# zhengfei0908/SBA-GAN

Hardware: AMD Instinct MI355X
Metric: images/sec (G+D step) at 256px (higher is better)
Workload: dtype bf16; 1 GPU; bird_style.yml 3-stage G+D step (64..256px), B=20 per GPU, G_NET variant=model, image_encoder=inception, text_encoder=RNN_ENCODER in the step; global_batch=20, parallelism=dp1, launch=replayer, losses_finite=True

## Files before the change

### include/sbagan_hip.h

```cpp
#ifndef SBAGAN_HIP_H
#define SBAGAN_HIP_H

#include <stdint.h>

#ifdef __cplusplus
extern "C" {
#endif

#define SBA_F32 0
#define SBA_BF16 1
#define SBA_BF16_YH 2

#define SBA_OK 0
#define SBA_E_ARG (-1)
#define SBA_E_LAUNCH (-2)
#define SBA_E_UNSUPPORTED (-3)

#define SBA_ACT_NONE 0
#define SBA_ACT_GLU 1
#define SBA_ACT_LRELU 2
#define SBA_ACT_RELU 3

#define SBA_MAX_TAPS 32

typedef struct sba_conv_geom {
    int32_t N, IH, IW, Cin;
    int32_t OH, OW, Cout;
    int32_t OHs, OWs;
    int32_t sy, sx;
    int32_t osy, osx, ooy, oox;
    int32_t ups;
    int32_t ntaps;
    int8_t ty[SBA_MAX_TAPS];
    int8_t tx[SBA_MAX_TAPS];
    int32_t x_cstride, x_coff, y_cstride, y_coff;
    int32_t relu;
    int32_t tile, ksplit;
    int32_t first_write;
    int32_t w_layout;
} sba_conv_geom;
#define SBA_IGEMM_TILES 18

const char* sba_version(void);

int sba_set_deterministic(int on, void* scratch, int64_t scratch_bytes);
int sba_get_deterministic(void);
int sba_det_reset(void);
int64_t sba_det_high_water(void);
int sba_set_reduce_scratch(void* scratch, int64_t scratch_bytes);
int sba_bn_stat_slots(void);

int sba_conv_igemm(int dtype, const void* x, const void* w, void* y, const void* addend,
                   float* stats, const sba_conv_geom* g, void* workspace, int64_t workspace_bytes,
                   void* stream);
int sba_conv_igemm_bias(int dtype, const void* x, const void* w, void* y, const void* addend,
                        float* stats, const float* bias, const void* relu_mask, const sba_conv_geom* g,
                        void* workspace, int64_t workspace_bytes, void* stream);
int sba_conv_igemm_plan(int dtype, const sba_conv_geom* g, int64_t workspace_bytes, int* plan);
int sba_conv_igemm_tile_shape(int tile, int* bm, int* bn);

int sba_fold_bn_pack(int dtype, const float* w, const float* gamma, const float* beta, const float* running_mean,
                     const float* running_var, float eps, void* out, float* bias, int O, int taps, int Cin, int glu,
                     void* stream);
int sba_conv_igemm_glu(int dtype, const void* x, const void* w, const float* bias, void* y, int C,
                       const sba_conv_geom* g, void* stream);
int sba_conv_igemm_glu_plan(int dtype, const sba_conv_geom* g, int C, int* plan);
#define SBA_GROUP_MAX 8
typedef struct sba_conv_group_item {
    const void* x; const void* w; void* y; const void* addend; const float* bias; const void* relu_mask;
    const sba_conv_geom* g;
} sba_conv_group_item;
int sba_conv_igemm_group(int dtype, int n, const sba_conv_group_item* items, int tile, void* stream);
int sba_conv_igemm_group_splitk(int dtype, int n, const sba_conv_group_item* items, int tile, int ksplit,
                                void* workspace, int64_t workspace_bytes, void* stream);
int sba_conv_wgrad(int dtype, const void* x, const void* dy, float* dw, const sba_conv_geom* g,
                   int ksplit, void* stream);
#define SBA_WGRAD_PLAN_INTS 14
int sba_conv_wgrad_plan(int dtype, const sba_conv_geom* g, int ksplit, int det, int* plan);
int sba_pack_weight(int dtype, const float* w, void* out, int Cout, int KH, int KW, int Cin,
                    int mode, void* stream);
typedef struct sba_pack_desc {
    const float* w;
    void* fwd;
    void* tr;
    int32_t Cout, KH, KW, Cin;
    int32_t mode;
    int32_t tile_begin;
    int32_t co_tiles, ci_tiles;
} sba_pack_desc;
int sba_pack_weights_multi(int dtype, const sba_pack_desc* descs, int ndesc, int total_tiles, void* stream);
typedef struct sba_frag_desc {
    const void* src;
    void* dst;
    int32_t R, taps, K, unit_begin;
} sba_frag_desc;
int sba_pack_frag_multi(const sba_frag_desc* descs, int ndesc, int total_units, void* stream);
int sba_pool2x2_sum(int dtype, const void* dup, void* dx, int N, int H, int W, int C, void* stream);

#ifndef SBA_BN_STAT_SLOTS
#define SBA_BN_STAT_SLOTS 8
#endif
int sba_bn_stats(int dtype, const void* y, float* stats, int64_t rows, int groups, int C, void* stream);
int sba_bn_act_fwd(int dtype, const void* y, const float* stats, const float* gamma, const float* beta,
                   float* running_mean, float* running_var, int64_t* num_batches_tracked, float* aux,
                   const void* residual, void* out, int64_t rows, int groups, int C, int act,
                   int out_cstride, int out_coff, float eps, float momentum, int training, void* stream);
int sba_bn_act_bwd_reduce(int dtype, const void* y, const void* dout, const float* aux, float* red,
                          int64_t rows, int groups, int C, int act, int dout_cstride, int dout_coff,
                          void* stream);
int sba_bn_act_bwd_apply(int dtype, const void* y, const void* dout, const float* aux, const float* red,
                         void* dy, float* dgamma, float* dbeta, int64_t rows, int groups, int C, int act,
                         int dout_cstride, int dout_coff, void* stream);
int sba_bn_act_fwd_fused(int dtype, const void* y, const float* gamma, const float* beta, float* running_mean,
                         float* running_var, int64_t* num_batches_tracked, float* aux, void* out, int64_t rows,
                         int groups, int C, int act, int out_cstride, int out_coff, float eps, float momentum,
                         void* stream);
int sba_bn_act_bwd_fused(int dtype, const void* y, const void* dout, const float* aux, void* dy,
                         float* dgamma, float* dbeta, int64_t rows, int groups, int C, int act,
                         int dout_cstride, int dout_coff, void* stream);
int sba_bn1d_glu_fwd(int dtype, const float* y, const float* gamma, const float* beta,
                     float* running_mean, float* running_var, int64_t* nbt, float* mean,
                     float* rstd, void* out, int B, int F, float eps, float momentum, void* stream);
int sba_bn1d_glu_bwd(int dtype, const float* y, const void* dout, const float* gamma,
                     const float* beta, const float* mean, const float* rstd, float* dy,
                     float* dgamma, float* dbeta, int B, int F, void* stream);

int sba_linear_fwd(const float* x, const float* w, const float* bias, float* y, int B, int K, int N,
                   void* stream);
int sba_linear_glu_fwd(int dtype, const float* x, const float* wp, const float* bias, void* out, int B, int K,
                       int F2, void* stream);
int sba_linear_bwd(const float* x, const float* w, const float* dy, float* dx, float* dw,
                   float* dbias, int B, int K, int N, void* stream);
int sba_ca_fwd(const float* h, const float* eps, float* c, float* mu, float* logvar, int B, int C,
               void* stream);
int sba_ca_bwd(const float* h, const float* eps, const float* dc, const float* dmu,
               const float* dlogvar, float* dh, int B, int C, void* stream);

int sba_ctx_proj_fwd(const float* words, const float* W, float* src, int B, int idf, int cdf, int L,
                     void* stream);
int sba_ctx_proj_fwd_fp8(const float* words, const float* W, float* src, int B, int idf, int cdf, int L,
                         void* stream);
int sba_ctx_proj_bwd(const float* words, const float* W, const float* dsrc, float* dW, float* dwords,
                     int B, int idf, int cdf, int L, void* stream);

int sba_instnorm_stats(int dtype, const void* h, float* mean, float* rstd, int N, int HW, int C,
                       float eps, void* stream);
int sba_adain_fwd(int dtype, const void* h, const float* mean, const float* rstd, const float* style,
                  void* out, int N, int HW, int C, int out_cstride, int out_coff, void* stream);
int sba_adain_bwd_reduce(int dtype, const void* h, const void* dout, const float* mean,
                         const float* rstd, float* red, int N, int HW, int C, int dout_cstride,
                         int dout_coff, void* stream);
int sba_adain_bwd_apply(int dtype, const void* h, const void* dout, const float* mean,
                        const float* rstd, const float* style, const float* red, void* dh,
                        float* dstyle, int N, int HW, int C, int dout_cstride, int dout_coff,
                        int accumulate, void* stream);

int sba_word_attn_fwd(int dtype, const void* h, const float* src, const uint8_t* mask, void* ctx,
                      float* att, int B, int Q, int idf, int L, int mask_mode, int out_cstride,
                      int out_coff, void* stream);
int sba_word_attn_fwd_fp8(const void* h, const float* src, const uint8_t* mask, void* ctx, float* att, int B, int Q,
                          int idf, int L, int mask_mode, int out_cstride, int out_coff, void* stream);
int sba_word_attn_bwd(int dtype, const void* h, const float* src, const uint8_t* mask,
                      const void* dctx, void* dh, float* dsrc, int B, int Q, int idf, int L,
                      int mask_mode, int dctx_cstride, int dctx_coff, int accumulate, void* stream);

int sba_img_head_fwd(int dtype, const void* h, const float* w, float* img, int N, int H, int W,
                     int C, void* stream);
int sba_img_head_bwd(int dtype, const void* h, const float* w, const float* img, const float* dimg,
                     void* dh, float* dw, int N, int H, int W, int C, int accumulate, void* stream);

int sba_d_stem_fwd(int dtype, const float* img, const float* w, void* out, int N, int S, int C,
                   void* stream);
int sba_d_stem_bwd(int dtype, const float* img, const float* w, const void* out, const void* dout,
                   float* dimg, float* dw, int N, int S, int C, void* stream);

int sba_logits_fwd(int dtype, const void* h, const float* w, const float* bias, float* prob, int B,
                   int K, void* stream);
int sba_logits_bwd(int dtype, const void* h, const float* w, const float* prob, const float* dprob,
                   void* dh, float* dw, float* dbias, int B, int K, int accumulate, void* stream);
int sba_cond_cat_fwd(int dtype, const void* h, const float* sent, void* out, int B, int C, int E,
                     void* stream);
int sba_cond_cat_bwd(int dtype, const void* dout, void* dh, float* dsent, int B, int C, int E,
                     int accumulate, void* stream);

int sba_resize_bilinear(const float* in, float* out, int NC, int S, int D, int backward, void* stream);
int sba_enc_stem_fwd(int dtype, const float* img, const float* w, const float* bias, void* out, int N, int S, int C,
                     void* stream);
int sba_enc_stem_bwd(int dtype, const float* w, const void* out, const void* dout, float* dimg, int N, int S, int C,
                     void* stream);
int sba_enc_stem_resize_fwd(int dtype, const float* img, const float* w, const float* bias, void* out, int N, int S, int D,
                            int C, void* stream);
int sba_maxpool3x3s2_fwd(int dtype, const void* x, void* y, int N, int H, int W, int C, int xcs, int xco, int ycs,
                         int yco, void* stream);
int sba_maxpool3x3s2_bwd(int dtype, const void* x, const void* dy, void* dx, int N, int H, int W, int C, int xcs,
                         int xco, int dycs, int dyco, int dxcs, int dxco, int accumulate, void* stream);
int sba_maxpool3x3s2_fwd_arg(int dtype, const void* x, void* y, uint8_t* argmax, int N, int H, int W, int C, int xcs,
                             int xco, int ycs, int yco, void* stream);
int sba_maxpool3x3s2_bwd_arg(int dtype, const uint8_t* argmax, const void* dy, void* dx, int N, int H, int W, int C,
                             int dycs, int dyco, int dxcs, int dxco, int accumulate, const void* relu_mask, void* stream);
int sba_avgpool3x3(int dtype, const void* x, void* y, int N, int H, int W, int C, int xcs, int xco, int ycs, int yco,
                   int accumulate, void* stream);
int sba_relu_bwd(int dtype, const void* out, const void* dout, void* dpre, int64_t rows, int C, int ocs, int oco,
                 int dcs, int dco, void* stream);
int sba_global_avgpool(int dtype, void* x, float* y, int N, int HW, int C, int backward, void* stream);
int sba_layout_nhwc_nchw(int dtype, void* nhwc, float* nchw, int N, int HW, int C, int to_nhwc, void* stream);

int sba_bce_multi(const float* prob, const int32_t* offsets, const float* target, const float* weight,
                  int nseg, float* loss, float* dprob, void* stream);
int sba_kl_loss(const float* mu, const float* logvar, float* loss, float* dmu, float* dlogvar,
                int n, void* stream);
int sba_damsm_words_fwd(const float* feat, const float* words, const int64_t* cap_lens, float* sim,
                        float* attn, float* attn1, float* wctx, int B, int nef, int R, int L,
                        float gamma1, float gamma2, void* stream);
int sba_damsm_words_bwd(const float* feat, const float* words, const int64_t* cap_lens,
                        const float* sim, const float* attn, const float* attn1, const float* wctx,
                        const float* dsim, float* dfeat, float* dwords, int B, int nef, int R, int L,
                        float gamma1, float gamma2, void* stream);
int64_t sba_damsm_prep_bytes(int B, int nef, int R, int L);
int64_t sba_damsm_bwd_bytes(int B, int nef, int R, int L);
int sba_damsm_prep(const float* feat, const float* words, const int64_t* cap_lens, void* prep, int64_t prep_bytes,
                   int B, int nef, int R, int L, void* stream);
int sba_damsm_words_fwd_mfma(const void* prep, const float* words, const int64_t* cap_lens, float* sim, float* attn,
                             float* attn1, float* wctx, int B, int nef, int R, int L, float gamma1, float gamma2,
                             void* stream);
int sba_damsm_words_bwd_mfma(const void* prep, const float* words, const int64_t* cap_lens, const float* sim,
                             const float* attn, const float* attn1, const float* wctx, const float* dsim,
                             void* scratch, int64_t scratch_bytes, float* dfeat, int accumulate, float* dwords,
                             int B, int nef, int R, int L, float gamma1, float gamma2, void* stream);
int sba_ce_pair_direct(const float* score, const uint8_t* mask, float scale, float lam, float* loss_out,
                       float* dscore, int B, void* stream);
int sba_damsm_sent_direct(const float* cnn, const float* rnn, const uint8_t* mask, float gamma3, float eps, float lam,
// ... 73 lines not shown
```

### sba-gan_amd/csrc/wgrad.hip

```cpp
#include "common.h"
#include "conv_common.h"

namespace {

struct FastDiv {
    uint64_t magic;
    uint32_t d;
};
static inline FastDiv make_fastdiv(uint32_t d, int64_t max_n) {
    FastDiv f;
    f.d = d;
    f.magic = (max_n < (1 << 21) && d > 0) ? (((uint64_t)1 << 42) + d - 1) / d : 0;
    return f;
}
__device__ __forceinline__ uint32_t fdiv(uint32_t n, const FastDiv& f) {
    return f.magic ? (uint32_t)(((uint64_t)n * f.magic) >> 42) : n / f.d;
}

__device__ __forceinline__ void zero_acc(f32x16_t (&acc)[2][2]) {
#pragma unroll
    for (int i = 0; i < 2; ++i)
#pragma unroll
        for (int j = 0; j < 2; ++j)
#pragma unroll
// ... 698 lines not shown
    for (int kw = 0; kw < 3; ++kw)
        store_tile<false>(acc[kw], dw + (int64_t)blockIdx.z * zstride, g, co0, ci0, kh * 3 + kw, mode, lane);
}

enum WgradFamily { WG_ROW_DMA = 0, WG_SMALL_DMA = 1, WG_SMALL = 2, WG_ROWS = 3, WG_GENERIC = 4 };

struct WgradPlan {
    int family;
    int v[4];
    dim3 grid;
    int block, lds;
    int per_split;
    int mode;
    int npart;
    int wclog;
};

static int pixel_splits(int target_wgs, int wgs, int chunks, int min_chunks, int* per_split) {
    int sp = cdiv(target_wgs, wgs);
    if (sp > chunks / min_chunks) sp = chunks / min_chunks > 0 ? chunks / min_chunks : 1;
    *per_split = cdiv(chunks, sp);
    return cdiv(chunks, *per_split);
}

static bool wgrad_plan(int dtype, const sba_conv_geom* g, int ksplit, bool det_on, WgradPlan* p) {
    if (!geom_ok(g, dtype)) return false;
    if (g->Cin % 8 != 0 || g->Cout % 8 != 0) return false;
    if (g->x_cstride || g->x_coff || g->y_cstride || g->y_coff || g->ntaps > 16) return false;
    const int M = g->N * g->OHs * g->OWs;
    if (ksplit < 1) ksplit = 1;
    const int fw = g->first_write ? 2 : 0;
    const int co_tiles = cdiv(g->Cout, 64), items = cdiv(g->Cin, 64) * g->ntaps;
    const bool dma_ok = dtype == SBA_BF16 && (int64_t)g->N * g->OH * g->OW * g->Cout * 2 < (1ll << 32);
    auto fill = [&](int family, int v0, int v1, int v2, int v3, dim3 grid, int block, int lds, int per_split, int unsplit_mode) {
        *p = WgradPlan{family, {v0, v1, v2, v3}, grid, block, lds, per_split, 0, 0, 0};
        const int nz = (int)grid.z;
        p->npart = det_on && (nz > 1 || family == WG_ROWS) ? nz : 0;
        p->mode = p->npart ? 2 : (nz > 1 ? 1 : unsplit_mode);
        return grid.y <= 65535 && grid.z <= 65535;
    };
    {
        const int kwn = g->ntaps == 16 ? 4 : (g->ntaps == 9 ? 3 : 0), sxy = g->sx;
        bool ok = dma_ok && kwn && g->sy == sxy && (!g->ups || kwn == 3) && g->osy == 1 && g->osx == 1 && g->ooy == 0 &&
                  g->oox == 0 && g->OHs == g->OH && g->OWs == g->OW && g->Cin % 64 == 0 && g->Cout % 64 == 0 &&
                  g->OW >= 4 && (g->OW & (g->OW - 1)) == 0 && !(g->OW == 4 && (g->ups || g->OH != 4)) && M % 32 == 0 &&
                  ((g->OH * g->OW) % 32 == 0 || g->OW == 4);
        ok = ok && ((kwn == 4 && sxy == 2) || (kwn == 3 && sxy == 1));
        for (int t = 0; t < g->ntaps && ok; ++t)
            ok = g->ty[t] == g->ty[(t / kwn) * kwn] && g->tx[t] == g->tx[(t / kwn) * kwn] + (t % kwn);
        if (ok) {
            const int wc = g->OW < 32 ? g->OW : 32;
            int wclog = 0;
            while ((1 << wclog) < wc) ++wclog;
            const int wgs = co_tiles * kwn * (g->Cin / 64);
            constexpr int ROW_WGS = 512;
            int cps32;
            const int sp = pixel_splits(wgs <= 8 ? (ROW_WGS * 3) / 4 : ROW_WGS, wgs, M / 32, 12, &cps32);
            const int xb = kwn == 4 ? 10 : (g->OW == 4 ? 6 : 5);
            const int stage = kwn == 4 ? WgRowCfg<4, 10>::STAGE : (g->OW == 4 ? WgRowCfg<3, 6>::STAGE : WgRowCfg<3, 5>::STAGE);
            if (fill(WG_ROW_DMA, kwn, sxy, xb, 4, dim3(co_tiles, kwn * (g->Cin / 64), sp), 64 * kwn, 4 * stage, cps32, fw)) {
                p->wclog = wclog;
                return true;
            }
        }
    }
    constexpr int SMALL_M = 12000;
    if (M <= SMALL_M && co_tiles * items >= 256) {
        const int wgs = co_tiles * cdiv(items, 4);
        constexpr int SMALL_WGS = 768, SMALL_MINC = 24;
        const int target = wgs >= SMALL_WGS / 2 ? wgs : SMALL_WGS;
        int cps;
        const int split = pixel_splits(target, wgs, cdiv(M, 16), SMALL_MINC, &cps);
        const dim3 grid(co_tiles, cdiv(items, 4), split);
        if (grid.y > 65535 || grid.z > 65535) return false;
        constexpr int DMA_WGS = 512;
        if (fw == 2 && wgs > DMA_WGS && g->Cout % 128 == 0 && dma_ok) {
            fill(WG_SMALL_DMA, 2, 3, 0, 0, dim3(co_tiles / 2, cdiv(items, 4), 1), 256, 3 * 6 * 32 * 128, cdiv(M, 32), fw);
            return true;
        }
        if (wgs <= DMA_WGS && dma_ok) {
            int cps32;
            const int sp = pixel_splits(target, wgs, cdiv(M, 32), SMALL_MINC / 2, &cps32);
            return fill(WG_SMALL_DMA, 1, 4, 0, 0, dim3(co_tiles, cdiv(items, 4), sp), 256, 4 * 5 * 32 * 128, cps32, fw);
        }
        return fill(WG_SMALL, dtype, 0, 0, 0, grid, 256, 0, cps, fw);
    }
    constexpr int ROWS_M = 131072;
    bool rows_ok = g->ntaps == 9 && g->sy == 1 && g->sx == 1 && g->osy == 1 && g->osx == 1 && g->ooy == 0 &&
                   g->oox == 0 && g->OHs == g->OH && g->OWs == g->OW && g->OW % 64 == 0 && M >= ROWS_M;
    for (int t = 0; t < 9 && rows_ok; ++t) rows_ok = g->ty[t] == t / 3 - 1 && g->tx[t] == t % 3 - 1;
    if (rows_ok) {
        const int ci_t = cdiv(g->Cin, 64);
        int spw;
        const int nz = pixel_splits(256, co_tiles * ci_t, g->N * g->OH * (g->OW / 64), 16, &spw);
        return fill(WG_ROWS, dtype, 0, 0, 0, dim3(co_tiles, ci_t, nz), 192, 0, spw, 1);
    }
    if (dma_ok) {
        constexpr int GEN_WGS = 512;
        int cps32;
        const int sp = pixel_splits(GEN_WGS, co_tiles * cdiv(items, 4), cdiv(M, 32), 12, &cps32);
        if (fill(WG_SMALL_DMA, 1, 4, 0, 0, dim3(co_tiles, cdiv(items, 4), sp), 256, 4 * 5 * 32 * 128, cps32, fw)) return true;
    }
    const int total_chunks = cdiv(M, 64);
    if (ksplit > total_chunks) ksplit = total_chunks;
    const int cps = cdiv(total_chunks, ksplit);
    return fill(WG_GENERIC, dtype, 0, 0, 0, dim3(co_tiles, items, cdiv(total_chunks, cps)), 256, 0, cps, 0);
}

template <auto Kernel, typename... Args>
static void launch_dyn_lds(const WgradPlan& p, hipStream_t st, Args... args) {
    static bool once = false;
    if (!once) { (void)hipFuncSetAttribute((const void*)Kernel, hipFuncAttributeMaxDynamicSharedMemorySize, p.lds); once = true; }
    SBA_LAUNCH(Kernel, p.grid, dim3(p.block), p.lds, st, args...);
}

static int wgrad_launch(const WgradPlan& p, int dtype, const void* x, const void* dy, float* dw, const sba_conv_geom* g,
                        hipStream_t st) {
    const int M = g->N * g->OHs * g->OWs;
    const FastDiv dsub = make_fastdiv((uint32_t)(g->OHs * g->OWs), (int64_t)M + 64);
    const FastDiv dow = make_fastdiv((uint32_t)g->OWs, (int64_t)M + 64);
    const int64_t dwn = (int64_t)g->Cout * g->ntaps * g->Cin;
    float* part = nullptr;
    if (p.npart) { part = sba_det_alloc((int64_t)p.npart * dwn); if (!part) return SBA_E_ARG; }
    float* dwa = part ? part : dw;
    const int64_t zs = part ? dwn : 0;
    const bf16_t* xh = (const bf16_t*)x;
    const bf16_t* dyh = (const bf16_t*)dy;
    switch (p.family) {
    case WG_ROW_DMA:
        if (p.v[0] == 4) launch_dyn_lds<wgrad_row_dma_kernel<4, 2, 10, 4>>(p, st, xh, dyh, dwa, *g, M, p.per_split, p.mode, dsub, dow, zs, p.wclog);
        else if (p.v[2] == 6) launch_dyn_lds<wgrad_row_dma_kernel<3, 1, 6, 4>>(p, st, xh, dyh, dwa, *g, M, p.per_split, p.mode, dsub, dow, zs, p.wclog);
        else launch_dyn_lds<wgrad_row_dma_kernel<3, 1, 5, 4>>(p, st, xh, dyh, dwa, *g, M, p.per_split, p.mode, dsub, dow, zs, p.wclog);
        break;
    case WG_SMALL_DMA:
        if (p.v[0] == 2) launch_dyn_lds<wgrad_small_dma_kernel<2, 3>>(p, st, xh, dyh, dwa, *g, M, p.per_split, p.mode, dsub, dow, zs);
        else launch_dyn_lds<wgrad_small_dma_kernel<1, 4>>(p, st, xh, dyh, dwa, *g, M, p.per_split, p.mode, dsub, dow, zs);
        break;
    case WG_SMALL:
        SBA_DISPATCH(dtype, SBA_LAUNCH((wgrad_small_kernel<T>), p.grid, dim3(p.block), 0, st, (const T*)x, (const T*)dy, dwa, *g, M,
                                       p.per_split, p.mode, dsub, dow, zs));
        break;
    case WG_ROWS:
        SBA_DISPATCH(dtype, SBA_LAUNCH((wgrad_rows_kernel<T>), p.grid, dim3(p.block), 0, st, (const T*)x, (const T*)dy, dwa, *g,
                                       g->N * g->OH * (g->OW / 64), p.per_split, p.mode, zs));
        break;
    default:
        SBA_DISPATCH(dtype, SBA_LAUNCH((wgrad_kernel<T>), p.grid, dim3(p.block), 0, st, (const T*)x, (const T*)dy, dwa, *g, M,
                                       p.per_split, p.mode, dsub, dow, zs));
    }
    if (part) sba_det_fold(part, 1, p.npart, dwn, dw, 0, g->first_write ? 1 : 0, st);
    return SBA_CHECK_LAUNCH();
}

}

extern "C" int sba_conv_wgrad_plan(int dtype, const sba_conv_geom* g, int ksplit, int det, int* plan) {
    WgradPlan p;
    if (!plan || !wgrad_plan(dtype, g, ksplit, det != 0, &p)) return SBA_E_ARG;
    const int out[SBA_WGRAD_PLAN_INTS] = {p.family, p.v[0], p.v[1], p.v[2], p.v[3], (int)p.grid.x, (int)p.grid.y, (int)p.grid.z,
                                          p.block, p.lds, p.per_split, p.mode, p.npart, p.wclog};
    for (int i = 0; i < SBA_WGRAD_PLAN_INTS; ++i) plan[i] = out[i];
    return SBA_OK;
}

extern "C" int sba_conv_wgrad(int dtype, const void* x, const void* dy, float* dw, const sba_conv_geom* g,
                              int ksplit, void* stream) {
    WgradPlan p;
    if (!x || !dy || !dw || !wgrad_plan(dtype, g, ksplit, sba_det_on(), &p)) return SBA_E_ARG;
    return wgrad_launch(p, dtype, x, dy, dw, g, (hipStream_t)stream);
}
```

### sba-gan_amd/sbagan/_lib.py

```python
import ctypes
import os

import torch
from ctypes import (POINTER, Structure, byref, c_char_p, c_float, c_int, c_int8, c_int32, c_int64,
                    c_uint64, c_void_p)

_HERE = os.path.dirname(os.path.abspath(__file__))
LIB_PATH = os.environ.get('SBA_LIB_PATH') or os.path.join(os.path.dirname(_HERE), 'csrc', 'libsbagan_hip.so')

SBA_F32, SBA_BF16, SBA_BF16_YH = 0, 1, 2
IGEMM_TILES = 18
WGRAD_PLAN_INTS = 14
WGRAD_FAMILIES = ('row_dma', 'small_dma', 'small', 'rows', 'generic')
ACT_NONE, ACT_GLU, ACT_LRELU, ACT_RELU = 0, 1, 2, 3
MAX_TAPS = 32


class ConvGeom(Structure):
    _fields_ = [('N', c_int32), ('IH', c_int32), ('IW', c_int32), ('Cin', c_int32),
                ('OH', c_int32), ('OW', c_int32), ('Cout', c_int32),
                ('OHs', c_int32), ('OWs', c_int32),
                ('sy', c_int32), ('sx', c_int32),
                ('osy', c_int32), ('osx', c_int32), ('ooy', c_int32), ('oox', c_int32),
                ('ups', c_int32), ('ntaps', c_int32),
                ('ty', c_int8 * MAX_TAPS), ('tx', c_int8 * MAX_TAPS),
                ('x_cstride', c_int32), ('x_coff', c_int32), ('y_cstride', c_int32), ('y_coff', c_int32),
                ('relu', c_int32), ('tile', c_int32), ('ksplit', c_int32), ('first_write', c_int32),
                ('w_layout', c_int32)]


class ConvGroupItem(Structure):
    _fields_ = [('x', c_void_p), ('w', c_void_p), ('y', c_void_p), ('addend', c_void_p), ('bias', c_void_p),
                ('relu_mask', c_void_p), ('g', POINTER(ConvGeom))]


GROUP_MAX = 8

if not os.path.exists(LIB_PATH):
    raise ImportError('libsbagan_hip.so not built: run `python __graft_entry__.py` or '
                      '`make -C sba-gan_amd/csrc` (expected %s)' % LIB_PATH)
lib = ctypes.CDLL(LIB_PATH)

P, I, F, L, U = c_void_p, c_int, c_float, c_int64, c_uint64
G = POINTER(ConvGeom)

SIGNATURES = {
    'sba_conv_igemm': [I, P, P, P, P, P, G, P, L, P],
    'sba_conv_igemm_bias': [I, P, P, P, P, P, P, P, G, P, L, P],
    'sba_conv_igemm_plan': [I, G, L, POINTER(c_int)],
    'sba_conv_igemm_tile_shape': [I, POINTER(c_int), POINTER(c_int)],
    'sba_fold_bn_pack': [I, P, P, P, P, P, F, P, P, I, I, I, I, P],
    'sba_conv_igemm_glu': [I, P, P, P, P, I, G, P],
    'sba_conv_igemm_glu_plan': [I, G, I, POINTER(c_int)],
    'sba_conv_igemm_group': [I, I, POINTER(ConvGroupItem), I, P],
    'sba_conv_igemm_group_splitk': [I, I, POINTER(ConvGroupItem), I, I, P, L, P],
    'sba_conv_wgrad': [I, P, P, P, G, I, P],
    'sba_conv_wgrad_plan': [I, G, I, I, POINTER(c_int)],
    'sba_pack_weight': [I, P, P, I, I, I, I, I, P],
    'sba_pack_frag_multi': [P, I, I, P],
    'sba_pack_weights_multi': [I, P, I, I, P],
    'sba_pool2x2_sum': [I, P, P, I, I, I, I, P],
    'sba_bn_stats': [I, P, P, L, I, I, P],
    'sba_bn_act_fwd': [I, P, P, P, P, P, P, P, P, P, P, L, I, I, I, I, I, F, F, I, P],
    'sba_bn_act_bwd_reduce': [I, P, P, P, P, L, I, I, I, I, I, P],
    'sba_bn_act_fwd_fused': [I, P, P, P, P, P, P, P, P, L, I, I, I, I, I, F, F, P],
    'sba_bn_act_bwd_fused': [I, P, P, P, P, P, P, L, I, I, I, I, I, P],
    'sba_bn_act_bwd_apply': [I, P, P, P, P, P, P, P, L, I, I, I, I, I, P],
    'sba_bn1d_glu_fwd': [I, P, P, P, P, P, P, P, P, P, I, I, F, F, P],
    'sba_bn1d_glu_bwd': [I, P, P, P, P, P, P, P, P, P, I, I, P],
    'sba_linear_fwd': [P, P, P, P, I, I, I, P],
    'sba_linear_glu_fwd': [I, P, P, P, P, I, I, I, P],
    'sba_linear_bwd': [P, P, P, P, P, P, I, I, I, P],
    'sba_ca_fwd': [P, P, P, P, P, I, I, P],
    'sba_ca_bwd': [P, P, P, P, P, P, I, I, P],
    'sba_ctx_proj_fwd': [P, P, P, I, I, I, I, P],
    'sba_ctx_proj_bwd': [P, P, P, P, P, I, I, I, I, P],
    'sba_ctx_proj_fwd_fp8': [P, P, P, I, I, I, I, P],
    'sba_instnorm_stats': [I, P, P, P, I, I, I, F, P],
    'sba_adain_fwd': [I, P, P, P, P, P, I, I, I, I, I, P],
    'sba_adain_bwd_reduce': [I, P, P, P, P, P, I, I, I, I, I, P],
    'sba_adain_bwd_apply': [I, P, P, P, P, P, P, P, P, I, I, I, I, I, I, P],
    'sba_word_attn_fwd': [I, P, P, P, P, P, I, I, I, I, I, I, I, P],
    'sba_word_attn_fwd_fp8': [P, P, P, P, P, I, I, I, I, I, I, I, P],
    'sba_word_attn_bwd': [I, P, P, P, P, P, P, I, I, I, I, I, I, I, I, P],
    'sba_img_head_fwd': [I, P, P, P, I, I, I, I, P],
    'sba_img_head_bwd': [I, P, P, P, P, P, P, I, I, I, I, I, P],
    'sba_d_stem_fwd': [I, P, P, P, I, I, I, P],
    'sba_d_stem_bwd': [I, P, P, P, P, P, P, I, I, I, P],
    'sba_logits_fwd': [I, P, P, P, P, I, I, P],
    'sba_logits_bwd': [I, P, P, P, P, P, P, P, I, I, I, P],
    'sba_cond_cat_fwd': [I, P, P, P, I, I, I, P],
    'sba_cond_cat_bwd': [I, P, P, P, I, I, I, I, P],
    'sba_resize_bilinear': [P, P, I, I, I, I, P],
    'sba_enc_stem_fwd': [I, P, P, P, P, I, I, I, P],
    'sba_enc_stem_resize_fwd': [I, P, P, P, P, I, I, I, I, P],
    'sba_enc_stem_bwd': [I, P, P, P, P, I, I, I, P],
    'sba_maxpool3x3s2_fwd': [I, P, P, I, I, I, I, I, I, I, I, P],
    'sba_maxpool3x3s2_bwd': [I, P, P, P, I, I, I, I, I, I, I, I, I, I, I, P],
    'sba_maxpool3x3s2_fwd_arg': [I, P, P, P, I, I, I, I, I, I, I, I, P],
    'sba_maxpool3x3s2_bwd_arg': [I, P, P, P, I, I, I, I, I, I, I, I, I, P, P],
    'sba_avgpool3x3': [I, P, P, I, I, I, I, I, I, I, I, I, P],
    'sba_relu_bwd': [I, P, P, P, L, I, I, I, I, I, P],
    'sba_global_avgpool': [I, P, P, I, I, I, I, P],
    'sba_layout_nhwc_nchw': [I, P, P, I, I, I, I, P],
    'sba_bce_multi': [P, P, P, P, I, P, P, P],
    'sba_kl_loss': [P, P, P, P, P, I, P],
    'sba_damsm_words_fwd': [P, P, P, P, P, P, P, I, I, I, I, F, F, P],
    'sba_damsm_words_bwd': [P, P, P, P, P, P, P, P, P, P, I, I, I, I, F, F, P],
    'sba_damsm_prep': [P, P, P, P, L, I, I, I, I, P],
    'sba_damsm_words_fwd_mfma': [P, P, P, P, P, P, P, I, I, I, I, F, F, P],
    'sba_damsm_words_bwd_mfma': [P, P, P, P, P, P, P, P, P, L, P, I, P, I, I, I, I, F, F, P],
    'sba_ce_pair_direct': [P, P, F, F, P, P, I, P],
    'sba_damsm_sent_direct': [P, P, P, F, F, F, P, P, I, I, P],
    'sba_damsm_sent_fwd': [P, P, P, I, I, F, F, P],
    'sba_damsm_sent_bwd': [P, P, P, P, P, I, I, F, F, P],
    'sba_ce_pair': [P, P, F, P, P, P, I, P],
    'sba_combine2': [P, P, P, P, P, I, P],
    'sba_adam_prepare': [P, F, F, F, P],
    'sba_adam_step': [P, P, P, P, P, P, P, L, F, F, F, F, P],
    'sba_cast': [I, P, I, P, L, P],
    'sba_lstm_bidir_fwd': [P, P, P, P, P, P, P, P, P, P, P, P, I, I, I, I, I, I, P],
    'sba_lstm_recur_train': [P, P, P, P, P, P, P, P, P, P, I, I, I, I, P],
    'sba_lstm_recur_bwd': [P, P, P, P, P, P, P, P, P, P, P, I, I, I, I, P],
    'sba_bert_embed_ln': [I, P, P, P, P, P, P, P, I, I, I, I, F, P],
    'sba_bert_add_ln': [I, P, P, P, P, P, I, I, F, P],
    'sba_bert_attention': [I, P, P, I, I, I, I, P],
    'sba_bert_gelu': [I, P, L, P],
    'sba_bert_tanh_transpose': [I, P, P, I, I, I, P],
    'sba_bert_embed_ln_train': [F, U, U, I, I, P, P, P, P, P, P, P, I, I, I, I, F, P],
    'sba_bert_add_ln_train': [F, U, U, I, I, P, P, P, P, P, I, I, F, P],
    'sba_bert_attention_train': [F, U, U, I, I, P, P, I, I, I, I, P],
    'sba_bert_words_head_bwd': [I, P, P, P, P, I, I, I, P],
    'sba_bert_sent_head_bwd': [P, P, P, P, P, P, P, P, P, P, I, I, I, P],
    'sba_rprec_rank': [P, P, P, P, F, P, P, I, I, I, I, P],
    'sba_vis_expand': [P, P, P, P, P, P, P, I, I, I, P],
    'sba_vis_compose': [P, I, I, I, I, I, I, I, P, P, P, P, I, P, I, I, P, I, I, P],
    'sba_fid_accumulate': [P, I, I, I, P, P, P],
    'sba_fid_finalize': [P, P, L, I, P, P, P, P],
    'sba_set_deterministic': [I, P, L],
    'sba_set_reduce_scratch': [P, L],
    'sba_det_reset': [],
    'sba_get_deterministic': [],
    'sba_bn_stat_slots': [],
    'sba_replay_create': [P, I, I, POINTER(c_void_p)],
    'sba_replay_launch': [P, P],
    'sba_replay_info': [P, POINTER(c_int)],
    'sba_replay_prioritize': [P, P, I, I, I, c_float, I],
    'sba_replay_marker': [I, P],
    'sba_replay_set_callback': [P, P, P],
    'sba_replay_destroy': [P],
}

for _name, _args in SIGNATURES.items():
    _fn = getattr(lib, _name)
    _fn.argtypes = _args
    _fn.restype = c_int
lib.sba_version.restype = c_char_p
lib.sba_version.argtypes = []
lib.sba_det_high_water.restype = c_int64
lib.sba_det_high_water.argtypes = []
lib.sba_damsm_prep_bytes.restype = c_int64
lib.sba_damsm_prep_bytes.argtypes = [I, I, I, I]
lib.sba_damsm_bwd_bytes.restype = c_int64
lib.sba_damsm_bwd_bytes.argtypes = [I, I, I, I]

_ERR = {-1: 'SBA_E_ARG (unsupported shape/alignment/enum)', -2: 'SBA_E_LAUNCH (HIP launch failed)',
        -3: 'SBA_E_UNSUPPORTED (graph node kind the replayer cannot re-issue)'}


AUDIT_HOOK = None


def call(name, *args):
    if AUDIT_HOOK is not None:
        AUDIT_HOOK(name, args)
    rc = getattr(lib, name)(*args)
    if rc != 0:
        raise RuntimeError('%s failed: %s' % (name, _ERR.get(rc, rc)))


def wgrad_plan(dtype, g, ksplit, det=None):
    plan = (c_int * WGRAD_PLAN_INTS)()
    det = lib.sba_get_deterministic() if det is None else int(det)
    call('sba_conv_wgrad_plan', dtype, byref(g), ksplit, det, plan)
    return list(plan)


def wgrad_plan_name(plan):
    fam, nargs = WGRAD_FAMILIES[plan[0]], (4, 2, 0, 0, 0)[plan[0]]
    args = ','.join(str(v) for v in plan[1:1 + nargs]) if nargs else ('f32', 'bf16')[plan[1]]
    return '%s<%s> x%d' % (fam, args, plan[7])


def version():
    return lib.sba_version().decode()
```

### sba-gan_amd/sbagan/ops.py

```python
import ctypes
import os
from collections import namedtuple

import torch

from . import _lib
from ._lib import ACT_GLU, ACT_LRELU, ACT_NONE, ConvGeom, call

CL = torch.channels_last
COMPUTE_DTYPE = torch.bfloat16
BN_EPS, BN_MOMENTUM, IN_EPS = 1e-5, 0.1, 1e-5

_WEIGHT_EPOCH = [0]


def set_compute_dtype(dt):
    global COMPUTE_DTYPE
    assert dt in (torch.bfloat16, torch.float32)
    COMPUTE_DTYPE = dt
    _WEIGHT_EPOCH[0] += 1


def compute_dtype():
    return COMPUTE_DTYPE
# ... 381 lines not shown
_IGEMM_TABLE = None


def geom_key(g):
    return '%d_%dx%d_%d_%dx%d_%d_t%d_s%d_u%d' % (g.N, g.IH, g.IW, g.Cin, g.OHs, g.OWs, g.Cout, g.ntaps, g.sy, g.ups)


_TABLE_FILE = None


def _table_section(name):
    global _TABLE_FILE
    if _TABLE_FILE is None:
        _TABLE_FILE = {}
        path = os.environ.get('SBA_IGEMM_TABLE_FILE') or os.path.join(os.path.dirname(os.path.abspath(__file__)),
                                                                      'igemm_table.json')
        if os.environ.get('SBA_IGEMM_TABLE', '1') != '0' and os.path.exists(path):
            import json
            with open(path) as f:
                _TABLE_FILE = json.load(f)
    return _TABLE_FILE.get(name, {})


def _igemm_table():
    global _IGEMM_TABLE
    if _IGEMM_TABLE is None:
        _IGEMM_TABLE = _table_section('bf16')
    return _IGEMM_TABLE


def tune_geom(g, dt):
    if getattr(g, '_tuned', None) != dt:
        g._tuned = dt
        ent = _igemm_table().get(geom_key(g)) if dt == _lib.SBA_BF16 else None
        g.tile, g.ksplit = (int(ent[0]), int(ent[1])) if ent else (0, 0)
    if IGEMM_LOG is not None:
        IGEMM_LOG.append(g)


def _igemm(dt, x, w, y, addend, stats, g, device, w_frag=None):
    ws = workspace(device)
    tune_geom(g, _lib.SBA_BF16 if dt == _lib.SBA_BF16_YH else dt)
    g.w_layout = 0
    if w_frag is not None and _halo_family(g):
        w, g.w_layout = w_frag.data_ptr(), 1
    try:
        call('sba_conv_igemm', dt, x, w, y, addend, stats, ctypes.byref(g), ws.data_ptr(), WORKSPACE_BYTES, _stream())
    finally:
        g.w_layout = 0


def _halo_family(g):
    h = getattr(g, '_halo', None)
    if h is None:
        plan = (ctypes.c_int * 3)()
        old = g.w_layout
        g.w_layout = 0
        call('sba_conv_igemm_plan', _lib.SBA_BF16, ctypes.byref(g), WORKSPACE_BYTES, plan)
        g.w_layout = old
        h = g._halo = plan[0] == 0
    return h




def conv_forward(x, pw, kind, want_stats=True, addend=None, pre_bn=False):
    _need_gpu(x)
    N, Cin, H, W = x.shape
    O = pw.param.shape[0]
    OH, OW = _conv_out_hw(kind, H, W)
    yh = pre_bn and Y_F16 and x.dtype == torch.bfloat16 and addend is None and O % 8 == 0
    if yh:
        y = torch.empty((N, O, OH, OW), dtype=torch.float16, device=x.device, memory_format=CL)
    else:
        y = empty_act(N, O, OH, OW, x)
    stats = zeros_f32((BN_STAT_SLOTS, 2 * O), x.device) if want_stats else None
    g = _geom((kind, N, H, W, Cin, O, None))
    wf = pw.fwd_frag(x.dtype) if kind == '3x3' else None
    _igemm(_lib.SBA_BF16_YH if yh else _dt(x), _p(x), _p(pw.fwd(x.dtype)), _p(y), _p(addend), _p(stats), g, x.device,
           w_frag=wf)
    return y, stats


def conv_dgrad(dy, pw, kind, in_hw, addend=None):
    N, O, OH, OW = dy.shape
    I = pw.param.shape[1]
    H, W = in_hw
    wd = pw.dgrad(dy.dtype, kind)
    if kind == '3x3':
        g = _geom(('3x3', N, OH, OW, O, I, None))
        dx = empty_act(N, I, H, W, dy)
        _igemm(_dt(dy), _p(dy), _p(wd), _p(dx), _p(addend), None, g, dy.device, w_frag=pw.dgrad_frag(dy.dtype, kind))
        return dx
    if kind == '3x3up':
        g = _geom(('4x4s2', N, OH, OW, O, I, None))
        dx = empty_act(N, I, H, W, dy)
        _igemm(_dt(dy), _p(dy), _p(wd), _p(dx), _p(addend), None, g, dy.device)
        return dx
    if kind == '4x4s2':
        dx = empty_act(N, I, H, W, dy)
        esz = dy.element_size()
        gs = [_geom(('4x4s2_dgrad', N, OH, OW, O, I, (cls // 2, cls % 2))) for cls in range(4)]
        if DGRAD4_GROUP and dy.dtype == torch.bfloat16 and O % 64 == 0:
            arr = (_lib.ConvGroupItem * 4)()
            for cls, (a, g) in enumerate(zip(arr, gs)):
                a.x, a.w, a.y, a.addend = _p(dy), wd.data_ptr() + cls * I * 4 * O * esz, _p(dx), _p(addend)
                a.bias = a.relu_mask = None
                a.g = ctypes.pointer(g)
            tile, split = dgrad4_plan(gs[0])
            ws = workspace(dy.device)
            call('sba_conv_igemm_group_splitk', _lib.SBA_BF16, 4, arr, tile, split, ws.data_ptr(), WORKSPACE_BYTES, _stream())
            if IGEMM_LOG is not None:
                IGEMM_LOG.append(('group', tile, gs))
            return dx
        for cls in range(4):
            wptr = wd.data_ptr() + cls * I * 4 * O * esz
            _igemm(_dt(dy), _p(dy), wptr, _p(dx), _p(addend), None, gs[cls], dy.device)
        return dx
    raise ValueError(kind)


DGRAD4_GROUP = True
_DGRAD4_FORCE = None


def dgrad4_plan(g):
    if _DGRAD4_FORCE:
        t, s = _DGRAD4_FORCE.split(',')
        return int(t), int(s)
    ent = _table_section('dgrad4').get(geom_key(g))
    if ent:
        return int(ent[0]), int(ent[1])
    M = g.N * g.OHs * g.OWs
    ny = (g.Cout + 63) // 64
    for tile, bm in ((5, 128), (3, 96), (1, 64)):
        tiles = 4 * ((M + bm - 1) // bm) * ny
        if tiles >= 512 or tile == 1:
            break
    ns64 = g.ntaps * (g.Cin // 64)
    split = max(1, min(512 // max(tiles, 1), ns64 // 8))
    return tile, split


_KSPLIT_TARGET = 640
_KSPLIT_MIN_CHUNKS = 24


def _ksplit(tiles, M):
    chunks = (M + 63) // 64
    want = max(1, (_KSPLIT_TARGET + tiles - 1) // tiles)
    return max(1, min(want, chunks // _KSPLIT_MIN_CHUNKS if chunks >= 2 * _KSPLIT_MIN_CHUNKS else 1))


def conv_wgrad(x, dy, param, kind):
    N, Cin, H, W = x.shape
    O = dy.shape[1]
    g = _geom((kind, N, H, W, Cin, O, None))
    gbuf = param_grad(param)
    M = N * g.OHs * g.OWs
    tiles = ((O + 63) // 64) * ((Cin + 63) // 64) * g.ntaps
    cell = getattr(param, '_sba_gepoch', None)
    first = 0
    if cell is not None and getattr(param, '_sba_wepoch', None) != cell[0]:
        param._sba_wepoch = cell[0]
        first = 1
    g.first_write = first
    call('sba_conv_wgrad', _dt(x), _p(x), _p(dy), _p(gbuf), ctypes.byref(g), _ksplit(tiles, M), _stream())


SIDE_WGRAD = False
HOME_STREAM = None
_COMPANION, _KEEPALIVE, _COMP_NEXT = {}, {}, {}
N_COMPANIONS = int(os.environ.get('SBA_WGRAD_COMPANIONS', '1'))


def _companion(device, *keep):
    cur = torch.cuda.current_stream()
    key = cur.cuda_stream
    comps = _COMPANION.get(key)
    if comps is None:
        comps = _COMPANION[key] = [torch.cuda.Stream(device=device) for _ in range(N_COMPANIONS)]
        _KEEPALIVE[key] = []
        _COMP_NEXT[key] = 0
    comp = comps[_COMP_NEXT[key] % len(comps)]
    _COMP_NEXT[key] += 1
    comp.wait_stream(cur)
    _KEEPALIVE[key].extend(keep)
    return comp


def conv_wgrad_overlapped(x, dy, param, kind):
    if not SIDE_WGRAD:
        return conv_wgrad(x, dy, param, kind)
    param_grad(param)
    with torch.cuda.stream(_companion(x.device, x, dy)):
        conv_wgrad(x, dy, param, kind)


def join_wgrads():
    cur = torch.cuda.current_stream()
    comps = _COMPANION.get(cur.cuda_stream)
    if comps is not None:
        for comp in comps:
            cur.wait_stream(comp)
        _KEEPALIVE[cur.cuda_stream].clear()
        _COMP_NEXT[cur.cuda_stream] = 0


def wgrad_tail_stream():
    cur = torch.cuda.current_stream()
    comps = _COMPANION.get(cur.cuda_stream)
    if comps is None:
        return cur
    comp = comps[0]
    comp.wait_stream(cur)
    for other in comps[1:]:
        comp.wait_stream(other)
    _KEEPALIVE[cur.cuda_stream].clear()
    _COMP_NEXT[cur.cuda_stream] = 0
    return comp


BN_STAT_SLOTS = _lib.lib.sba_bn_stat_slots()


_DET_SCRATCH = [None]
DET_SCRATCH_BYTES = int(os.environ.get('SBA_DET_SCRATCH_MB', '2048')) << 20


def set_deterministic(flag, device=None):
    if torch.cuda.is_available():
        torch.cuda.synchronize()
    if flag:
        dev = torch.device('cuda', torch.cuda.current_device()) if device is None else device
        if _DET_SCRATCH[0] is None or _DET_SCRATCH[0].device != dev:
            _DET_SCRATCH[0] = torch.empty(DET_SCRATCH_BYTES, dtype=torch.uint8, device=dev)
        call('sba_set_deterministic', 1, _DET_SCRATCH[0].data_ptr(), DET_SCRATCH_BYTES)
    else:
        call('sba_set_deterministic', 0, None, 0)


def deterministic():
    return bool(_lib.lib.sba_get_deterministic())


def det_reset():
    if _lib.lib.sba_get_deterministic():
        call('sba_det_reset')


if os.environ.get('SBA_DETERMINISTIC', '0') == '1' and torch.cuda.is_available():
    set_deterministic(True)


class BNState(object):
    __slots__ = ('aux', 'C', 'rows', 'groups')


def bn_act_forward(y, stats, bn, act, residual=None, groups=1):
    N, C, H, W = y.shape
    Co = C // 2 if act == ACT_GLU else C
    st = BNState()
    st.C, st.rows, st.groups = C, (N // groups) * H * W, groups
    st.aux = torch.empty((groups, 4, C), dtype=torch.float32, device=y.device)
    out = torch.empty((N, Co, H, W), dtype=_act_dtype(y), device=y.device, memory_format=CL)
    call('sba_bn_act_fwd', _dt(y), _p(y), _p(stats), _p(bn.weight), _p(bn.bias), _p(bn.running_mean),
         _p(bn.running_var), _p(bn.num_batches_tracked), _p(st.aux), _p(residual), _p(out), st.rows, groups, C,
         act, Co, 0, BN_EPS, BN_MOMENTUM, 1 if bn.training else 0, _stream())
    return out, st


BN_FUSED_BWD_ROWS = 2560


def bn_act_backward(y, dout, st, bn, act, need_param_grad=True, out=None, red=None):
    N, C, H, W = y.shape
    Co = C // 2 if act == ACT_GLU else C
    dy = out if out is not None else torch.empty(y.shape, dtype=_act_dtype(y), device=y.device, memory_format=CL)
    dg = db = None
    if need_param_grad:
        dg, db = param_grad(bn.weight), param_grad(bn.bias)
    if st.rows <= BN_FUSED_BWD_ROWS:
        call('sba_bn_act_bwd_fused', _dt(y), _p(y), _p(dout), _p(st.aux), _p(dy), _p(dg), _p(db), st.rows, st.groups,
             C, act, Co, 0, _stream())
        return dy
    if red is None:
        red = zeros_f32((st.groups, BN_STAT_SLOTS, 2 * C), y.device)
        call('sba_bn_act_bwd_reduce', _dt(y), _p(y), _p(dout), _p(st.aux), _p(red), st.rows, st.groups, C, act, Co, 0,
             _stream())
    call('sba_bn_act_bwd_apply', _dt(y), _p(y), _p(dout), _p(st.aux), _p(red), _p(dy), _p(dg), _p(db), st.rows,
         st.groups, C, act, Co, 0, _stream())
    return dy


def bn_act_forward_fused(y, bn, act, groups):
    N, C, H, W = y.shape
    Co = C // 2 if act == ACT_GLU else C
    st = BNState()
    st.C, st.rows, st.groups = C, (N // groups) * H * W, groups
    st.aux = torch.empty((groups, 4, C), dtype=torch.float32, device=y.device)
    out = torch.empty((N, Co, H, W), dtype=_act_dtype(y), device=y.device, memory_format=CL)
    call('sba_bn_act_fwd_fused', _dt(y), _p(y), _p(bn.weight), _p(bn.bias), _p(bn.running_mean), _p(bn.running_var),
         _p(bn.num_batches_tracked), _p(st.aux), _p(out), st.rows, groups, C, act, Co, 0, BN_EPS, BN_MOMENTUM, _stream())
    return out, st


def bn_stats(y, groups=1):
    N, C, H, W = y.shape
    stats = zeros_f32((groups, BN_STAT_SLOTS, 2 * C), y.device)
    call('sba_bn_stats', _dt(y), _p(y), _p(stats), (N // groups) * H * W, groups, C, _stream())
    return stats


def bn_act_forward_grouped(y, bn, act, groups):
    N, C, H, W = y.shape
    if bn.training and (N // groups) * H * W <= BN_FUSED_BWD_ROWS:
        return bn_act_forward_fused(y, bn, act, groups)
    stats = bn_stats(y, groups) if bn.training else None
    return bn_act_forward(y, stats, bn, act, None, groups)
# ... 1152 lines not shown
```

Baseline: 2099 images/sec.

## Collapse upsample-fused 3x3 conv weight-gradient into a stride-2 4x4 wgrad plus unfold

For a 3x3 conv applied after a nearest 2x upsample, the weight gradient is computed on the low-resolution grid. It runs as a stride-2, 16-tap correlation of dy against x into an fp32 scratch, which avoids iterating over the 4x larger upsampled pixel grid. A small unfold kernel then sums 2x2 groups of the 16 taps into the 9 taps of the real 3x3 kernel and transposes them into the dw layout, then zeroes the scratch. This adds a workspace dependency and an extra kernel launch. It applies only when the derived plan maps to the row-DMA family and the pixel count clears a threshold; otherwise it falls back to the direct path.

```diff
diff --git a/include/sbagan_hip.h b/include/sbagan_hip.h
--- a/include/sbagan_hip.h
+++ b/include/sbagan_hip.h
@@ -77,6 +77,11 @@
                    int ksplit, void* stream);
 #define SBA_WGRAD_PLAN_INTS 14
 int sba_conv_wgrad_plan(int dtype, const sba_conv_geom* g, int ksplit, int det, int* plan);
+int sba_conv_wgrad_ups(int dtype, const void* x, const void* dy, float* dw, const sba_conv_geom* g, int ksplit,
+                       void* ws, int64_t ws_bytes, int path, void* stream);
+#define SBA_WGRAD_UPS_PLAN_INTS 16
+int sba_conv_wgrad_ups_plan(int dtype, const sba_conv_geom* g, int ksplit, int det, int64_t ws_bytes, int path,
+                            sba_conv_geom* derived, int64_t* scratch_bytes, int* plan);
 int sba_pack_weight(int dtype, const float* w, void* out, int Cout, int KH, int KW, int Cin,
                     int mode, void* stream);
 typedef struct sba_pack_desc {
diff --git a/sba-gan_amd/csrc/wgrad.hip b/sba-gan_amd/csrc/wgrad.hip
--- a/sba-gan_amd/csrc/wgrad.hip
+++ b/sba-gan_amd/csrc/wgrad.hip
@@ -874,6 +874,131 @@
     return SBA_CHECK_LAUNCH();
 }
 
+__global__ __launch_bounds__(256) void wgrad_ups_unfold_kernel(float* __restrict__ G, float* __restrict__ dw, const int Cin,
+                                                               const int Cout, const int store) {
+    __shared__ float tile[9][32][33];
+    const int tid = threadIdx.x, r = tid >> 3, c4 = (tid & 7) * 4;
+    const int co0 = blockIdx.x * 32, ci0 = blockIdx.y * 32;
+    float* gp = G + (int64_t)(ci0 + r) * 16 * Cout + co0 + c4;
+    float4 v[16];
+#pragma unroll
+    for (int s = 0; s < 16; ++s) v[s] = *reinterpret_cast<const float4*>(gp + (int64_t)s * Cout);
+#pragma unroll
+    for (int s = 0; s < 16; ++s) *reinterpret_cast<float4*>(gp + (int64_t)s * Cout) = make_float4(0.f, 0.f, 0.f, 0.f);
+#pragma unroll
+    for (int kh = 0; kh < 3; ++kh)
+#pragma unroll
+        for (int kw = 0; kw < 3; ++kw) {
+            const float4 a = v[(2 - kh) * 4 + 2 - kw], b = v[(2 - kh) * 4 + 3 - kw];
+            const float4 c = v[(3 - kh) * 4 + 2 - kw], d = v[(3 - kh) * 4 + 3 - kw];
+            float* t = &tile[kh * 3 + kw][r][c4];
+            t[0] = ((a.x + b.x) + c.x) + d.x;
+            t[1] = ((a.y + b.y) + c.y) + d.y;
+            t[2] = ((a.z + b.z) + c.z) + d.z;
+            t[3] = ((a.w + b.w) + c.w) + d.w;
+        }
+    __syncthreads();
+#pragma unroll
+    for (int t = 0; t < 9; ++t) {
+        float4 o = make_float4(tile[t][c4][r], tile[t][c4 + 1][r], tile[t][c4 + 2][r], tile[t][c4 + 3][r]);
+        float4* p = reinterpret_cast<float4*>(dw + ((int64_t)(co0 + r) * 9 + t) * Cin + ci0 + c4);
+        if (!store) {
+            const float4 old = *p;
+            o.x += old.x; o.y += old.y; o.z += old.z; o.w += old.w;
+        }
+        *p = o;
+    }
+}
+
+enum WgradUpsReason { UPS_COLLAPSED = 0, UPS_DIRECT_ASKED = 1, UPS_NOT_ELIGIBLE = 2, UPS_NO_SCRATCH = 3, UPS_BELOW_THRESHOLD = 4 };
+
+struct WgradUpsPlan {
+    int collapsed, reason;
+    sba_conv_geom d;
+    int64_t scratch;
+    WgradPlan p;
+};
+
+static bool ups_derive(const sba_conv_geom* g, sba_conv_geom* d) {
+    *d = sba_conv_geom{};
+    if (!g || !g->ups || g->ntaps != 9 || g->sy != 1 || g->sx != 1 || g->IH <= 0 || g->IW <= 0 || g->OH != 2 * g->IH ||
+        g->OW != 2 * g->IW || g->OHs != g->OH || g->OWs != g->OW || g->osy != 1 || g->osx != 1 || g->ooy || g->oox)
+        return false;
+    for (int t = 0; t < 9; ++t)
+        if (g->ty[t] != t / 3 - 1 || g->tx[t] != t % 3 - 1) return false;
+    d->N = g->N;
+    d->IH = g->OH; d->IW = g->OW; d->Cin = g->Cout;
+    d->OH = d->OHs = g->IH; d->OW = d->OWs = g->IW; d->Cout = g->Cin;
+    d->sy = d->sx = 2;
+    d->osy = d->osx = 1;
+    d->ntaps = 16;
+    for (int t = 0; t < 16; ++t) { d->ty[t] = (int8_t)(t / 4 - 1); d->tx[t] = (int8_t)(t % 4 - 1); }
+    d->x_cstride = g->y_cstride; d->x_coff = g->y_coff;
+    d->y_cstride = g->x_cstride; d->y_coff = g->x_coff;
+    d->first_write = 1;
+    return true;
+}
+
+static bool ups_collapse_pays(const sba_conv_geom* g) {
+    constexpr int64_t UPS_MIN_PIXELS = 1024;
+    return (int64_t)g->N * g->IH * g->IW >= UPS_MIN_PIXELS;
+}
+
+static bool wgrad_ups_plan(int dtype, const sba_conv_geom* g, int ksplit, bool det_on, int64_t ws_bytes, int path,
+                           WgradUpsPlan* u) {
+    u->collapsed = 0;
+    u->scratch = 0;
+    const bool ups3 = ups_derive(g, &u->d);
+    if (ups3) u->scratch = (int64_t)g->Cin * 16 * g->Cout * 4;
+    u->reason = UPS_NOT_ELIGIBLE;
+    if (path == 1) u->reason = UPS_DIRECT_ASKED;
+    else if (ups3 && geom_ok(g, dtype)) {
+        if (wgrad_plan(dtype, &u->d, 1, det_on, &u->p) && u->p.family == WG_ROW_DMA) {
+            if (u->scratch > ws_bytes) u->reason = UPS_NO_SCRATCH;
+            else if (path == 0 && !ups_collapse_pays(g)) u->reason = UPS_BELOW_THRESHOLD;
+            else u->reason = UPS_COLLAPSED;
+        }
+    }
+    u->collapsed = u->reason == UPS_COLLAPSED;
+    if (u->collapsed) return true;
+    if (path == 2) return false;
+    return wgrad_plan(dtype, g, ksplit, det_on, &u->p);
+}
+
+}
+
+extern "C" int sba_conv_wgrad_ups_plan(int dtype, const sba_conv_geom* g, int ksplit, int det, int64_t ws_bytes, int path,
+                                       sba_conv_geom* derived, int64_t* scratch_bytes, int* plan) {
+    if (!plan || path < 0 || path > 2) return SBA_E_ARG;
+    WgradUpsPlan u;
+    const bool ok = wgrad_ups_plan(dtype, g, ksplit, det != 0, ws_bytes, path, &u);
+    if (derived) *derived = u.d;
+    if (scratch_bytes) *scratch_bytes = u.scratch;
+    plan[0] = u.collapsed;
+    plan[1] = u.reason;
+    for (int i = 2; i < SBA_WGRAD_UPS_PLAN_INTS; ++i) plan[i] = -1;
+    if (!ok) return SBA_E_ARG;
+    const WgradPlan& p = u.p;
+    const int out[SBA_WGRAD_PLAN_INTS] = {p.family, p.v[0], p.v[1], p.v[2], p.v[3], (int)p.grid.x, (int)p.grid.y, (int)p.grid.z,
+                                          p.block, p.lds, p.per_split, p.mode, p.npart, p.wclog};
+    for (int i = 0; i < SBA_WGRAD_PLAN_INTS; ++i) plan[2 + i] = out[i];
+    return SBA_OK;
+}
+
+extern "C" int sba_conv_wgrad_ups(int dtype, const void* x, const void* dy, float* dw, const sba_conv_geom* g, int ksplit,
+                                  void* ws, int64_t ws_bytes, int path, void* stream) {
+    if (!x || !dy || !dw || path < 0 || path > 2) return SBA_E_ARG;
+    if (!ws || ((uintptr_t)ws & 15) != 0) ws_bytes = 0;
+    WgradUpsPlan u;
+    if (!wgrad_ups_plan(dtype, g, ksplit, sba_det_on(), ws_bytes, path, &u)) return SBA_E_ARG;
+    hipStream_t st = (hipStream_t)stream;
+    if (!u.collapsed) return wgrad_launch(u.p, dtype, x, dy, dw, g, st);
+    float* G = (float*)ws;
+    const int rc = wgrad_launch(u.p, dtype, dy, x, G, &u.d, st);
+    if (rc != SBA_OK) return rc;
+    SBA_LAUNCH(wgrad_ups_unfold_kernel, dim3(g->Cout / 32, g->Cin / 32), dim3(256), 0, st, G, dw, g->Cin, g->Cout,
+               g->first_write ? 1 : 0);
+    return SBA_CHECK_LAUNCH();
 }
 
 extern "C" int sba_conv_wgrad_plan(int dtype, const sba_conv_geom* g, int ksplit, int det, int* plan) {
diff --git a/sba-gan_amd/sbagan/_lib.py b/sba-gan_amd/sbagan/_lib.py
--- a/sba-gan_amd/sbagan/_lib.py
+++ b/sba-gan_amd/sbagan/_lib.py
@@ -56,6 +56,8 @@
     'sba_conv_igemm_group_splitk': [I, I, POINTER(ConvGroupItem), I, I, P, L, P],
     'sba_conv_wgrad': [I, P, P, P, G, I, P],
     'sba_conv_wgrad_plan': [I, G, I, I, POINTER(c_int)],
+    'sba_conv_wgrad_ups': [I, P, P, P, G, I, P, L, I, P],
+    'sba_conv_wgrad_ups_plan': [I, G, I, I, L, I, G, POINTER(c_int64), POINTER(c_int)],
     'sba_pack_weight': [I, P, P, I, I, I, I, I, P],
     'sba_pack_frag_multi': [P, I, I, P],
     'sba_pack_weights_multi': [I, P, I, I, P],
@@ -186,6 +188,19 @@
     return list(plan)
 
 
+WGRAD_UPS_PLAN_INTS = 16
+WGRAD_UPS_AUTO, WGRAD_UPS_DIRECT, WGRAD_UPS_COLLAPSED = 0, 1, 2
+WGRAD_UPS_REASONS = ('collapsed', 'direct asked', 'not eligible', 'workspace too small', 'below threshold')
+
+
+def wgrad_ups_plan(dtype, g, ksplit, ws_bytes, path=0, det=None):
+    plan = (c_int * WGRAD_UPS_PLAN_INTS)()
+    d, nbytes = ConvGeom(), c_int64(0)
+    det = lib.sba_get_deterministic() if det is None else int(det)
+    rc = lib.sba_conv_wgrad_ups_plan(dtype, byref(g), ksplit, det, ws_bytes, path, byref(d), byref(nbytes), plan)
+    return rc, plan[0], plan[1], d, nbytes.value, list(plan[2:])
+
+
 def wgrad_plan_name(plan):
     fam, nargs = WGRAD_FAMILIES[plan[0]], (4, 2, 0, 0, 0)[plan[0]]
     args = ','.join(str(v) for v in plan[1:1 + nargs]) if nargs else ('f32', 'bf16')[plan[1]]
diff --git a/sba-gan_amd/sbagan/ops.py b/sba-gan_amd/sbagan/ops.py
--- a/sba-gan_amd/sbagan/ops.py
+++ b/sba-gan_amd/sbagan/ops.py
@@ -557,6 +557,9 @@
     return max(1, min(want, chunks // _KSPLIT_MIN_CHUNKS if chunks >= 2 * _KSPLIT_MIN_CHUNKS else 1))
 
 
+WGRAD_UPS_PATH = 0
+
+
 def conv_wgrad(x, dy, param, kind):
     N, Cin, H, W = x.shape
     O = dy.shape[1]
@@ -570,6 +573,11 @@
         param._sba_wepoch = cell[0]
         first = 1
     g.first_write = first
+    if kind == '3x3up':
+        ws = workspace(x.device)
+        call('sba_conv_wgrad_ups', _dt(x), _p(x), _p(dy), _p(gbuf), ctypes.byref(g), _ksplit(tiles, M), ws.data_ptr(),
+             WORKSPACE_BYTES, WGRAD_UPS_PATH, _stream())
+        return
     call('sba_conv_wgrad', _dt(x), _p(x), _p(dy), _p(gbuf), ctypes.byref(g), _ksplit(tiles, M), _stream())
 
 
```

New measurement: 2111 images/sec (median of 6 runs). No clear change (+0.6%).
